# xrouting/xroute_env

Hardware: AMD Instinct MI355X
Metric: env-steps/sec (batched regions), ispd18_test1-sized regions (higher is better)
Workload: dtype u32 distances / i16 state / fp32 observation

## Files before the change

### xroute_env_amd/csrc/xr_kernels.hip

```cpp
#include <hip/hip_runtime.h>
#include <stdint.h>
#include <initializer_list>
#include <type_traits>

#include "xr_device.h"
#include "../../include/xroute_hip.h"

#define XR_FNV_PRIME 0x100000001b3ULL

__device__ __forceinline__ void fnv_mix(uint64_t& h, uint32_t w) { h = (h ^ (uint64_t)w) * XR_FNV_PRIME; }

__device__ __forceinline__ uint64_t splitmix64(uint64_t x) {
    x += 0x9E3779B97F4A7C15ULL;
    uint64_t z = x;
    z = (z ^ (z >> 30)) * 0xBF58476D1CE4E5B9ULL;
    z = (z ^ (z >> 27)) * 0x94D049BB133111EBULL;
    return z ^ (z >> 31);
}

__global__ void xr_ingest_kernel(const uint32_t* __restrict__ rec, int16_t* __restrict__ node_net,
                                 int16_t* __restrict__ owner0, int64_t total) {
    int64_t i = (int64_t)blockIdx.x * blockDim.x + threadIdx.x;
    const int64_t stride = (int64_t)gridDim.x * blockDim.x;
    for (; i < total; i += stride) {
// ... 1044 lines not shown
    __syncthreads();
    uint32_t v = 0, incl = 0;
    if (t < 256) {
        v = s_cnt[255 - t];
        incl = v;
        for (int o = 1; o < 64; o <<= 1) {
            const uint32_t u = __shfl_up(incl, o, 64);
            if ((t & 63) >= o) incl += u;
        }
        if ((t & 63) == 63) s_wsum[t >> 6] = incl;
    }
    __syncthreads();
    if (t < 256) {
        uint32_t base = 0;
        for (int w = 0; w < (t >> 6); w++) base += s_wsum[w];
        s_cnt[255 - t] = base + incl - v;
    }
    __syncthreads();
#pragma unroll
    for (int k = 0; k < 8; k++)
        if (cls[k] >= 0) order[atomicAdd(&s_cnt[cls[k]], 1u)] = e0 + t + k * 1024;
    for (int e = e0 + t + 8 * 1024; e < e1; e += 1024) order[atomicAdd(&s_cnt[xr_route_work_class(b, actions, e)], 1u)] = e;
}

template <bool LDS_DIST, int ZCH>
__global__ void __launch_bounds__(1024, 4) xr_route_kernel(XrBatchDev b, const int32_t* __restrict__ actions) {
    extern __shared__ __attribute__((aligned(16))) char smem[];
#ifdef XR_TIMELINE
    if (threadIdx.x == 0) {
        b.phase_cycles[(int64_t)blockIdx.x * 8 + 0] = (long long)wall_clock64();
        b.phase_cycles[(int64_t)blockIdx.x * 8 + 3] = (long long)__smid();
    }
#endif
    const int e_ = b.route_order ? b.route_order[blockIdx.x] : (int)blockIdx.x + b.env_base;
    xr_route_dispatch<LDS_DIST, ZCH>(b, e_, actions[e_], smem);
#ifdef XR_TIMELINE
    if (threadIdx.x == 0) b.phase_cycles[(int64_t)blockIdx.x * 8 + 1] = (long long)wall_clock64();
#endif
    if (b.obs_out) xr_obs_epilogue(b, e_, smem, b.obs_head_only != 0);
#ifdef XR_TIMELINE
    __syncthreads();
    if (threadIdx.x == 0) b.phase_cycles[(int64_t)blockIdx.x * 8 + 2] = (long long)wall_clock64();
#endif
}

template <int BT>
__global__ void __launch_bounds__(BT) xr_plan_kernel(XrBatchDev b, const int32_t* __restrict__ actions, uint32_t* __restrict__ next_queue,
                                                     int32_t* __restrict__ order) {
    __shared__ int s_wsum[BT / 64];
    __shared__ int s_base;
    const int tid = threadIdx.x, lane = tid & 63, wv = tid >> 6;
    const int e = b.env_base + blockIdx.x * BT + tid, e_end = XR_ENV_END(b);
    if (blockIdx.x == 0 && tid < 3 && next_queue) next_queue[tid] = 0u;
    int k = 0, r = 0;
    const uint64_t* lsrc = nullptr;
    int clear_bit = -1;
    bool was_reset = false;
    if (e < e_end) {
        const int nl = b.nlegal[e];
        r = b.env_region[e];
        was_reset = (nl == 0);
        if (nl == 0) {
            if (b.auto_reset) {
                if (b.env_replay[e] == b.max_route_count) r = (int)(((int64_t)r + b.n_envs) % b.n_regions);
                const XrRegionDev R = b.regions[r];
                lsrc = b.legal0 + R.legal0_off;
                k = R.nlegal0;
            }
        } else {
            const XrRegionDev R = b.regions[r];
            const int a = actions[e];
            lsrc = b.legal + (int64_t)e * b.legal_words;
            k = nl;
            if (a >= 1 && a <= R.n_nets && ((lsrc[(a - 1) >> 6] >> ((a - 1) & 63)) & 1ULL)) {
                clear_bit = a - 1;
                k = nl - 1;
            }
        }
        b.plan_region[e] = r;
    }
    int kskip = XR_SPLIT_KEEP(b, k);
    if (b.obs_incremental && e < e_end && !was_reset) {
        if (clear_bit < 0) kskip = k;
        else {
            int below = 0;
            for (int w = 0; w <= (clear_bit >> 6); w++) {
                uint64_t m = lsrc[w];
                if (w == (clear_bit >> 6)) m &= (1ULL << (clear_bit & 63)) - 1ULL;
                below += __popcll(m);
            }
            kskip = below;
        }
    }
    const int kw = k - kskip;
    int incl = kw;
#pragma unroll
    for (int d = 1; d < 64; d <<= 1) {
        const int t = __shfl_up(incl, d, 64);
        if (lane >= d) incl += t;
    }
    if (lane == 63) s_wsum[wv] = incl;
    __syncthreads();
    int woff = 0;
    for (int w = 0; w < wv; w++) woff += s_wsum[w];
    if (tid == BT - 1) s_base = (int)atomicAdd(&b.queue[2], (unsigned)(woff + incl));
    __syncthreads();
    const int off = s_base + woff + incl - kw;
    if (e < e_end) {
        int j = 0;
        for (int w = 0; w < b.legal_words && j < k; w++) {
            uint64_t m = lsrc[w];
            if (clear_bit >= 0 && (clear_bit >> 6) == w) m &= ~(1ULL << (clear_bit & 63));
            while (m) {
                const int bit = __ffsll((unsigned long long)m) - 1;
                m &= m - 1;
                if (j >= kskip) {
                    b.plan_units[off + j - kskip] = ((uint32_t)e << 14) | (uint32_t)j;
                    b.plan_unit_net[off + j - kskip] = (w << 6) + bit + 1;
                }
                j++;
            }
        }
    }
    if (order) {
        __shared__ uint32_t s_cnt[256];
        __shared__ uint32_t s_csum[4];
        if (tid < 256) s_cnt[tid] = 0;
        __syncthreads();
        const int cls = e < e_end ? xr_route_work_class(b, actions, e) : -1;
        if (cls >= 0) atomicAdd(&s_cnt[cls], 1u);
        __syncthreads();
        uint32_t v = 0, inc = 0;
        if (tid < 256) {
            v = s_cnt[255 - tid];
            inc = v;
            for (int o = 1; o < 64; o <<= 1) {
                const uint32_t u = __shfl_up(inc, o, 64);
                if (lane >= o) inc += u;
            }
            if (lane == 63) s_csum[wv] = inc;
        }
        __syncthreads();
        if (tid < 256) {
            uint32_t base = 0;
            for (int w = 0; w < wv; w++) base += s_csum[w];
            s_cnt[255 - tid] = base + inc - v;
        }
        __syncthreads();
        if (cls >= 0) order[atomicAdd(&s_cnt[cls], 1u)] = e;
    }
}

#define XR_NP_J 9
template <int J = XR_NP_J>
__device__ __forceinline__ void xr_unit_aligned(const XrBatchDev& b, int u, int t_lo = 0, int t_hi = 1 << 22) {
    const int tid = threadIdx.x;
    const uint32_t ent = b.plan_units[u];
    const int id = b.plan_unit_net[u];
    const int e = (int)(ent >> 14), rank = (int)(ent & 0x3FFFu);
    const XrRegionDev R = b.regions[b.plan_region[e]];
    const int N = R.N, Z = R.Z, Y = R.Y, X = R.X, YZ = Y * Z;
    const int16_t* __restrict__ nn = b.rg_node_net + R.node_off;
    float* __restrict__ out = b.obs_out + (int64_t)e * b.obs_stride + (int64_t)(2 + 7 * rank) * N;
    const int ngrp = N >> 2;
    const int ap_lo = b.net_csr[R.net_off + id], ap_hi = b.net_csr[R.net_off + id + 1];
    (void)nn; (void)X; (void)Y; (void)Z; (void)YZ;
    const int gend = min(ngrp, t_hi << 8);
    for (int g0 = t_lo << 8; g0 < gend; g0 += 256 * J) {
        unsigned bits[J];
#pragma unroll
        for (int j = 0; j < J; j++) bits[j] = 0;
        for (int i = ap_lo; i < ap_hi; i++) {
            const int v = b.ap_feat[R.ap_off + i];
            const int f = v & 0x7FFFFFFF;
            const unsigned m = (1u | (v < 0 ? 16u : 0u)) << (f & 3);
            const int g = (f >> 2) - g0 - tid;
#pragma unroll
            for (int j = 0; j < J; j++) bits[j] |= (g == j * 256) ? m : 0u;
        }
#pragma unroll
        for (int j = 0; j < J; j++) {
            const int g = g0 + j * 256 + tid;
            if (g < gend) {
                float* __restrict__ pp = out + ((int64_t)g << 2);
                const unsigned m0 = bits[j], m1 = bits[j] >> 4;
                float4 v0, v1;
                v0.x = (m0 & 1u) ? 1.f : 0.f; v0.y = (m0 & 2u) ? 1.f : 0.f; v0.z = (m0 & 4u) ? 1.f : 0.f; v0.w = (m0 & 8u) ? 1.f : 0.f;
                v1.x = (m1 & 1u) ? 1.f : 0.f; v1.y = (m1 & 2u) ? 1.f : 0.f; v1.z = (m1 & 4u) ? 1.f : 0.f; v1.w = (m1 & 8u) ? 1.f : 0.f;
                XR_ST4(pp, v0);
#pragma unroll
                for (int pl = 1; pl < 7; pl++) XR_ST4(pp + (int64_t)pl * N, v1);
            }
        }
    }
}

__global__ void __launch_bounds__(256) xr_netplane_kernel(XrBatchDev b) {
    const int total = (int)b.queue[2];
    for (int u = blockIdx.x; u < total; u += gridDim.x) xr_unit_aligned(b, u);
}

__device__ __forceinline__ void xr_unit_stream(const XrBatchDev& b, int u, uint32_t* s_m) {
    const int tid = threadIdx.x;
    const uint32_t ent = b.plan_units[u];
    const int id = b.plan_unit_net[u];
    const int e = (int)(ent >> 14), rank = (int)(ent & 0x3FFFu);
    const XrRegionDev R = b.regions[b.plan_region[e]];
    const int N = R.N, Z = R.Z, Y = R.Y, X = R.X, YZ = Y * Z;
    const int nwords = (N + 15) >> 4;
    (void)X; (void)Y; (void)Z; (void)YZ;
    const int ap_lo = b.net_csr[R.net_off + id], ap_hi = b.net_csr[R.net_off + id + 1];
    int my_ap = 0;
    const bool has_ap = ap_lo + tid < ap_hi;
    if (has_ap) my_ap = b.ap_feat[R.ap_off + ap_lo + tid];
    for (int w = tid; w <= nwords; w += 256) s_m[w] = 0u;
    xr_lds_barrier();
    if (has_ap) {
        const int f = my_ap & 0x7FFFFFFF;
        atomicOr(&s_m[f >> 4], (my_ap < 0 ? 3u : 1u) << ((f & 15) << 1));
    }
    xr_lds_barrier();
    float* __restrict__ run = b.obs_out + (int64_t)e * b.obs_stride + (int64_t)(2 + 7 * rank) * N;
    const int total = 7 * N;
    const int head = (int)((32u - (uint32_t)((reinterpret_cast<uintptr_t>(run) >> 2) & 31u)) & 31u);
    const int nslot = total > head ? (total - head) >> 2 : 0;
    const int piece = ((nslot + 7 * 256 - 1) / (7 * 256)) * 256;
    auto one = [&](int o) -> float {
        int pl = 0, f = o;
        while (f >= N) { f -= N; pl++; }
        return ((s_m[f >> 4] >> (((f & 15) << 1) + (pl ? 1 : 0))) & 1u) ? 1.f : 0.f;
    };
    int ppl[7], pnd[7];
#pragma unroll
    for (int p = 0; p < 7; p++) {
        int o = head + ((p * piece + tid) << 2), pl = 0;
        while (o >= N && pl < 7) { o -= N; pl++; }
        ppl[p] = pl; pnd[p] = o;
    }
    for (int it = 0; it < piece; it += 256) {
#pragma unroll
        for (int p = 0; p < 7; p++) {
            const int sl = p * piece + it + tid;
            if (sl < nslot) {
                const int f = pnd[p], pl = ppl[p];
                float4 v;
                if (f + 3 < N) {
                    const int bit = f << 1, w = bit >> 5;
                    const uint32_t m = __funnelshift_r(s_m[w], s_m[w + 1], bit & 31) >> (pl ? 1 : 0);
                    v.x = (m & 1u) ? 1.f : 0.f; v.y = (m & 4u) ? 1.f : 0.f; v.z = (m & 16u) ? 1.f : 0.f; v.w = (m & 64u) ? 1.f : 0.f;
                } else {
                    const int o = head + (sl << 2);
                    v.x = one(o); v.y = one(o + 1); v.z = one(o + 2); v.w = one(o + 3);
                }
                XR_ST4(run + head + (sl << 2), v);
            }
            int nf = pnd[p] + 1024;
            while (nf >= N) { nf -= N; ppl[p]++; }
            pnd[p] = nf;
        }
    }
    if (tid < head && tid < total) run[tid] = one(tid);
    const int tail0 = head + (nslot << 2);
    if (tid >= 64 && tail0 + (tid - 64) < total) run[tail0 + (tid - 64)] = one(tail0 + (tid - 64));
    xr_lds_barrier();
}

typedef unsigned xr_u4 __attribute__((ext_vector_type(4)));
#define XR_STU8(ptr, v) __builtin_nontemporal_store((v), reinterpret_cast<xr_u4*>(ptr))
__device__ __forceinline__ uint32_t xr_nib_bytes(uint32_t m) {
    return (m & 1u) | ((m & 2u) << 7) | ((m & 4u) << 14) | ((m & 8u) << 21);
}
__device__ __forceinline__ xr_u4 xr_bits_bytes16(uint32_t m) {
    return xr_u4{xr_nib_bytes(m), xr_nib_bytes(m >> 4), xr_nib_bytes(m >> 8), xr_nib_bytes(m >> 12)};
}
__device__ __forceinline__ uint32_t xr_pair_bytes(uint32_t m) {
    return (m & 1u) | ((m & 4u) << 6) | ((m & 16u) << 12) | ((m & 64u) << 18);
}
__device__ __forceinline__ uint32_t xr_obst_bytes4(uint32_t n0, uint32_t n1, uint32_t w0, uint32_t w1) {
    auto ob = [](uint32_t n, uint32_t w) -> uint32_t { return ((n & 0xFFFFu) == 0xFFFFu || (w & 0xFFFFu) != 0u) ? 1u : 0u; };
    return ob(n0, w0) | (ob(n0 >> 16, w0 >> 16) << 8) | (ob(n1, w1) << 16) | (ob(n1 >> 16, w1 >> 16) << 24);
}

__device__ __forceinline__ void xr_obs_head_u8(const XrBatchDev& b, int e, char* smem) {
    __syncthreads();
    const XrRegionDev R = b.regions[b.env_region[e]];
    int* s_ids = reinterpret_cast<int*>(smem);
    int* s_pref = s_ids + b.legal_words * 64;
    const int tid = threadIdx.x, nthr = (int)blockDim.x;
    int K;
    if (b.legal_words <= nthr) {
        const uint64_t my_m = tid < b.legal_words ? b.legal[(int64_t)e * b.legal_words + tid] : 0ull;
        K = xr_legal_ids_pre(my_m, b.legal_words, s_ids, s_pref);
    } else {
        K = xr_legal_ids(b.legal + (int64_t)e * b.legal_words, b.legal_words, s_ids, s_pref);
    }
    const int16_t* __restrict__ nn = b.rg_node_net + R.node_off;
    const int16_t* __restrict__ ow = b.owner + (int64_t)e * b.n_max;
    uint8_t* __restrict__ out = b.obs_out_u8 + (int64_t)e * b.obs_stride;
    const int N = R.N, total = 2 * N, nslot = total >> 4;
    auto one = [&](int o) -> uint32_t {
        if (o < N) return (nn[o] == -1 || ow[o] != 0) ? 1u : 0u;
        return o - N < K ? ((uint32_t)s_ids[o - N] & 0xFFu) : 0u;
    };
    for (int s = tid; s < nslot; s += nthr) {
        const int o = s << 4;
        xr_u4 v;
        if (o + 16 <= N) {
            const int4 a0 = *reinterpret_cast<const int4*>(nn + o), a1 = *reinterpret_cast<const int4*>(nn + o + 8);
            const int4 c0 = *reinterpret_cast<const int4*>(ow + o), c1 = *reinterpret_cast<const int4*>(ow + o + 8);
            v = xr_u4{xr_obst_bytes4(a0.x, a0.y, c0.x, c0.y), xr_obst_bytes4(a0.z, a0.w, c0.z, c0.w),
                      xr_obst_bytes4(a1.x, a1.y, c1.x, c1.y), xr_obst_bytes4(a1.z, a1.w, c1.z, c1.w)};
        } else if (o >= N + K) {
            v = xr_u4{0u, 0u, 0u, 0u};
        } else {
            uint32_t w[4];
#pragma unroll
            for (int q = 0; q < 4; q++)
                w[q] = one(o + 4 * q) | (one(o + 4 * q + 1) << 8) | (one(o + 4 * q + 2) << 16) | (one(o + 4 * q + 3) << 24);
            v = xr_u4{w[0], w[1], w[2], w[3]};
        }
        XR_STU8(out + o, v);
    }
    const int tail0 = nslot << 4;
    if (tid < total - tail0) out[tail0 + tid] = (uint8_t)one(tail0 + tid);
}

#define XR_NPU8_J 4
__device__ __forceinline__ void xr_unit_u8_aligned(const XrBatchDev& b, int u) {
    const int tid = threadIdx.x, nthr = (int)blockDim.x;
    const uint32_t ent = b.plan_units[u];
    const int id = b.plan_unit_net[u];
    const int e = (int)(ent >> 14), rank = (int)(ent & 0x3FFFu);
    const XrRegionDev R = b.regions[b.plan_region[e]];
    const int N = R.N;
    uint8_t* __restrict__ out = b.obs_out_u8 + (int64_t)e * b.obs_stride + (int64_t)(2 + 7 * rank) * N;
    const int ngrp = N >> 4;
    const int ap_lo = b.net_csr[R.net_off + id], ap_hi = b.net_csr[R.net_off + id + 1];
    for (int g0 = 0; g0 < ngrp; g0 += nthr * XR_NPU8_J) {
        uint32_t bits[XR_NPU8_J];
#pragma unroll
        for (int j = 0; j < XR_NPU8_J; j++) bits[j] = 0;
        for (int i = ap_lo; i < ap_hi; i++) {
            const int v = b.ap_feat[R.ap_off + i];
            const int f = v & 0x7FFFFFFF;
            const uint32_t m = (1u | (v < 0 ? 0x10000u : 0u)) << (f & 15);
            const int g = (f >> 4) - g0 - tid;
#pragma unroll
            for (int j = 0; j < XR_NPU8_J; j++) bits[j] |= (g == j * nthr) ? m : 0u;
        }
#pragma unroll
        for (int j = 0; j < XR_NPU8_J; j++) {
            const int g = g0 + j * nthr + tid;
            if (g < ngrp) {
                uint8_t* __restrict__ pp = out + ((int64_t)g << 4);
                const xr_u4 v0 = xr_bits_bytes16(bits[j]), v1 = xr_bits_bytes16(bits[j] >> 16);
                XR_STU8(pp, v0);
#pragma unroll
                for (int pl = 1; pl < 7; pl++) XR_STU8(pp + (int64_t)pl * N, v1);
            }
        }
    }
}

__device__ __forceinline__ void xr_unit_u8_stream(const XrBatchDev& b, int u, uint32_t* s_m) {
    const int tid = threadIdx.x, nthr = (int)blockDim.x;
    const uint32_t ent = b.plan_units[u];
    const int id = b.plan_unit_net[u];
    const int e = (int)(ent >> 14), rank = (int)(ent & 0x3FFFu);
    const XrRegionDev R = b.regions[b.plan_region[e]];
    const int N = R.N;
    const int nwords = (N + 15) >> 4;
    const int ap_lo = b.net_csr[R.net_off + id], ap_hi = b.net_csr[R.net_off + id + 1];
    for (int w = tid; w <= nwords; w += nthr) s_m[w] = 0u;
    xr_lds_barrier();
    for (int i = ap_lo + tid; i < ap_hi; i += nthr) {
        const int v = b.ap_feat[R.ap_off + i];
        const int f = v & 0x7FFFFFFF;
        atomicOr(&s_m[f >> 4], (v < 0 ? 3u : 1u) << ((f & 15) << 1));
    }
    xr_lds_barrier();
    uint8_t* __restrict__ run = b.obs_out_u8 + (int64_t)e * b.obs_stride + (int64_t)(2 + 7 * rank) * N;
    const int total = 7 * N;
    const int head = min(total, (int)((128u - (uint32_t)(reinterpret_cast<uintptr_t>(run) & 127u)) & 127u));
    const int nslot = (total - head) >> 4;
    auto one = [&](int o) -> uint32_t {
        const int pl = o / N, f = o - pl * N;
        return (s_m[f >> 4] >> (((f & 15) << 1) + (pl ? 1 : 0))) & 1u;
    };
    for (int sl = tid; sl < nslot; sl += nthr) {
        const int o = head + (sl << 4);
        const int pl = o / N, f = o - pl * N;
        xr_u4 v;
        if (f + 15 < N) {
            const int bit = f << 1, w = bit >> 5;
            const uint32_t m = __funnelshift_r(s_m[w], s_m[w + 1], bit & 31) >> (pl ? 1 : 0);
            v = xr_u4{xr_pair_bytes(m), xr_pair_bytes(m >> 8), xr_pair_bytes(m >> 16), xr_pair_bytes(m >> 24)};
        } else {
            uint32_t q4[4];
#pragma unroll
            for (int q = 0; q < 4; q++)
                q4[q] = one(o + 4 * q) | (one(o + 4 * q + 1) << 8) | (one(o + 4 * q + 2) << 16) | (one(o + 4 * q + 3) << 24);
            v = xr_u4{q4[0], q4[1], q4[2], q4[3]};
        }
        XR_STU8(run + o, v);
    }
    for (int i = tid; i < head; i += nthr) run[i] = (uint8_t)one(i);
    const int tail0 = head + (nslot << 4);
    for (int i = tail0 + tid; i < total; i += nthr) run[i] = (uint8_t)one(i);
    xr_lds_barrier();
}

__global__ void __launch_bounds__(256) xr_obs_u8_kernel(XrBatchDev b, uint8_t* __restrict__ out, int64_t env_stride, int env_lo) {
    extern __shared__ __attribute__((aligned(16))) char smem[];
    int* s_ids = reinterpret_cast<int*>(smem);
    int* s_pref = s_ids + b.legal_words * 64;
    const int e = env_lo + blockIdx.y;
    const XrRegionDev R = b.regions[b.env_region[e]];
    const int N = R.N;
    const int64_t slot0 = (int64_t)blockIdx.x * blockDim.x;
    if ((slot0 << 4) >= (int64_t)(2 + 7 * (int64_t)R.n_nets) * N) return;
    const int K = xr_legal_ids(b.legal + (int64_t)e * b.legal_words, b.legal_words, s_ids, s_pref);
    const int64_t total = (int64_t)(2 + 7 * (int64_t)K) * N;
    const int64_t o = (slot0 + threadIdx.x) << 4;
    if (o >= total) return;
    XrStateSrc src{b.rg_node_net + R.node_off, b.owner + (int64_t)e * b.n_max};
    uint8_t* __restrict__ row = out + (int64_t)blockIdx.y * env_stride;
    int p = (int)(o / N), f = (int)(o - (int64_t)p * N);
    uint32_t w[4] = {0u, 0u, 0u, 0u};
    const int cnt = total - o < 16 ? (int)(total - o) : 16;
    for (int j = 0; j < cnt; j++) {
        float obst; int apnet; bool adj;
        xr_node_features(src, f, R.X, R.Y, R.Z, N, obst, apnet, adj);
        uint32_t v;
        if (p == 0) v = obst != 0.f ? 1u : 0u;
        else if (p == 1) v = f < K ? ((uint32_t)s_ids[f] & 0xFFu) : 0u;
        else {
            const int pi = p - 2, i = pi / 7, c = pi - 7 * i;
            v = (apnet != 0 && apnet == s_ids[i] && (c == 0 || adj)) ? 1u : 0u;
        }
        w[j >> 2] |= v << ((j & 3) << 3);
        if (++f == N) { f = 0; ++p; }
    }
    if (cnt == 16) {
        XR_STU8(row + o, (xr_u4{w[0], w[1], w[2], w[3]}));
    } else {
        for (int j = 0; j < cnt; j++) row[o + j] = (uint8_t)(w[j >> 2] >> ((j & 3) << 3));
    }
}

constexpr int XR_QUEUE_BATCH = 1;
constexpr int XR_TICKET_TILES = 3;
static_assert(XR_TICKET_TILES >= 1 && XR_TICKET_TILES <= XR_NP_J, "a slab is one pass of xr_unit_aligned");
__device__ __forceinline__ void xr_queue_first(int G, int sh, int& first_r, int& first_u) {
    if (sh < 0) { first_r = G; first_u = 0; return; }
    first_r = ((G >> (sh + 1)) << sh) + min(G & ((2 << sh) - 1), 1 << sh);
    first_u = G - first_r;
}

__global__ void __launch_bounds__(256) xr_unit_helper_kernel(XrBatchDev b) {
    __shared__ int s_u;
    const int total = (int)b.queue[2];
    int first_r, first_u;
    xr_queue_first(b.queue_grid, b.queue_skip_shift, first_r, first_u);
    for (;;) {
        if (threadIdx.x == 0) s_u = first_u + (int)atomicAdd(&b.queue[1], 1u);
        __syncthreads();
        const int u = s_u;
        __syncthreads();
        if (u >= total) break;
        xr_unit_aligned(b, u);
    }
}

__global__ void __launch_bounds__(256) xr_netplane_stream_kernel(XrBatchDev b) {
    extern __shared__ __attribute__((aligned(16))) char smem[];
    const int total = (int)b.queue[2];
    for (int u = blockIdx.x; u < total; u += gridDim.x) xr_unit_stream(b, u, reinterpret_cast<uint32_t*>(smem));
}

constexpr int XR_QUEUE_WAVES_PER_SIMD = 4;
template <bool LDS_DIST, int ZCH, bool U8>
__device__ __forceinline__ void xr_step_queue_body(XrBatchDev& b, const int32_t* __restrict__ actions, char* smem) {
    __shared__ int s_task;
    const int tid = threadIdx.x;
    const int B = XR_ENV_END(b) - b.env_base;
    const int units = (int)b.queue[2];
    int S = 1;
    if (!U8 && b.obs_vec4 == 1 && b.queue_slab_tickets) {
        S = ((b.n_max + 1023) / 1024 + XR_TICKET_TILES - 1) / XR_TICKET_TILES;
        if ((int64_t)units * S > 0x7FF00000LL) S = 1;
    }
    const int total = units * S;
    const bool claim_late = S > 1;
    const int quota = S * max(1, (int)(((int64_t)units * b.queue_quota_pm) / (1000 * (int64_t)B)));
    bool routes_left = true, units_left = total > 0;
    bool skip_route = b.queue_skip_shift >= 0 && ((blockIdx.x >> b.queue_skip_shift) & 1) != 0;
    int first_r = 0, first_u = 0, my_first = -1;
    const bool unit_first = skip_route;
    {
        const int sh = b.queue_skip_shift, G = (int)gridDim.x, i = (int)blockIdx.x;
        xr_queue_first(G, sh, first_r, first_u);
        my_first = sh < 0 ? i : ((i >> (sh + 1)) << sh) + (i & ((1 << sh) - 1));
    }
#ifdef XR_TIMELINE
    long long tl_start = wall_clock64(), tl_route = 0, tl_unit = 0, tl_last_route = 0;
    int tl_nr = 0, tl_nu = 0;
#define XR_TL_NOW() wall_clock64()
#endif
    while (routes_left || units_left) {
        if (routes_left && !skip_route) {
            if (tid == 0) {
                const int t = (my_first >= 0 && !unit_first) ? my_first : first_r + (int)atomicAdd(&b.queue[0], 1u);
                s_task = (t < B && b.route_order) ? b.route_order[t] : b.env_base + t;
            }
            if (!unit_first) my_first = -1;
            xr_lds_barrier();
            const int e = s_task;
            xr_lds_barrier();
            if (e < b.env_base + B) {
#ifdef XR_TIMELINE
                const long long t0 = XR_TL_NOW();
#endif
                xr_route_dispatch<LDS_DIST, ZCH>(b, e, actions[e], smem);
                if constexpr (U8) xr_obs_head_u8(b, e, smem);
                else xr_obs_epilogue(b, e, smem, true);
                xr_lds_barrier();
#ifdef XR_TIMELINE
                tl_last_route = XR_TL_NOW(); tl_route += tl_last_route - t0; tl_nr++;
#endif
            } else {
                routes_left = false;
            }
        }
        skip_route = false;
        if (units_left) {
            const int nb = routes_left ? max(1, quota / XR_QUEUE_BATCH) : (1 << 30);
            unsigned nx = 0;
            const unsigned ubase = (unsigned)first_u * (unsigned)XR_QUEUE_BATCH;
            auto claim = [&]() -> unsigned { return ubase + atomicAdd(&b.queue[1], (unsigned)XR_QUEUE_BATCH); };
            if (tid == 0) nx = (my_first >= 0 && unit_first) ? (unsigned)my_first * (unsigned)XR_QUEUE_BATCH : claim();
            if (unit_first) my_first = -1;
            for (int i = 0; i < nb; i++) {
                if (tid == 0) s_task = (int)nx;
                xr_lds_barrier();
                const int u0 = s_task;
                xr_lds_barrier();
                if (u0 >= total) { units_left = false; break; }
                if (!claim_late && tid == 0 && i + 1 < nb) nx = claim();
#ifdef XR_TIMELINE
                const long long t0 = XR_TL_NOW();
#endif
                const int u1 = min(u0 + XR_QUEUE_BATCH, total);
                for (int u = u0; u < u1; u++) {
                    if constexpr (U8) {
                        if (b.obs_vec4 == 1) xr_unit_u8_aligned(b, u);
                        else xr_unit_u8_stream(b, u, reinterpret_cast<uint32_t*>(smem));
                    } else {
                        if (b.obs_vec4 == 1) {
                            if (S > 1) {
                                const int uu = u / S, p = u - uu * S;
                                xr_unit_aligned<XR_TICKET_TILES>(b, uu, p * XR_TICKET_TILES, (p + 1) * XR_TICKET_TILES);
                            } else xr_unit_aligned(b, u);
                        } else xr_unit_stream(b, u, reinterpret_cast<uint32_t*>(smem));
                    }
                }
#ifdef XR_TIMELINE
                tl_unit += XR_TL_NOW() - t0; tl_nu += u1 - u0;
#endif
                if (claim_late && tid == 0 && i + 1 < nb) nx = claim();
            }
            xr_lds_barrier();
        }
    }
#ifdef XR_TIMELINE
    if (tid == 0 && (int)blockIdx.x < B) {
        long long* o = b.phase_cycles + (int64_t)blockIdx.x * 8;
        o[0] = tl_start; o[1] = XR_TL_NOW(); o[2] = tl_route; o[3] = tl_unit; o[4] = tl_nr; o[5] = tl_nu; o[6] = tl_last_route; o[7] = 1;
    }
#endif
}

template <bool LDS_DIST, int ZCH>
__global__ void __launch_bounds__(1024, XR_QUEUE_WAVES_PER_SIMD) xr_step_queue_kernel(XrBatchDev b, const int32_t* __restrict__ actions) {
    extern __shared__ __attribute__((aligned(16))) char smem[];
    xr_step_queue_body<LDS_DIST, ZCH, false>(b, actions, smem);
}

template <bool LDS_DIST, int ZCH>
__global__ void __launch_bounds__(1024, XR_QUEUE_WAVES_PER_SIMD) xr_step_queue_u8_kernel(XrBatchDev b, const int32_t* __restrict__ actions) {
    extern __shared__ __attribute__((aligned(16))) char smem[];
    xr_step_queue_body<LDS_DIST, ZCH, true>(b, actions, smem);
}

template <bool LDS_DIST, int ZCH>
__global__ void xr_order_kernel(XrBatchDev b, const int32_t* __restrict__ orders, int stride,
                                int32_t* __restrict__ net_stats) {
    extern __shared__ __attribute__((aligned(16))) char smem[];
    const int e = blockIdx.x;
    const int tid = threadIdx.x;
    xr_env_reset(b, e, 0, 0);
    __syncthreads();
    int st_acc = 0, plen_acc = 0, sweeps_acc = 0;
    const int32_t* __restrict__ ord = orders + (int64_t)e * stride;
    for (int k = 0; k < stride; k++) {
        const int a = ord[k];
// ... 265 lines not shown
    hipError_t e = hipFuncGetAttributes(&attr, fn);
    if (e != hipSuccess) return e;
    *static_lds = attr.sharedSizeBytes;
    return hipOccupancyMaxActiveBlocksPerMultiprocessor(wg_per_cu, fn, v.threads, v.lds_bytes);
}

hipError_t xr_launch_step_queue(const XrBatchDev* b, const int32_t* actions, XrRouteVariant v, int blocks, hipStream_t st) {
    const dim3 g(blocks), t(v.threads);
    xr_with_variant(v.lds_dist, v.zch, [&](auto L, auto Z) {
        if (b->obs_out_u8) hipLaunchKernelGGL((xr_step_queue_u8_kernel<L.value, Z.value>), g, t, v.lds_bytes, st, *b, actions);
        else hipLaunchKernelGGL((xr_step_queue_kernel<L.value, Z.value>), g, t, v.lds_bytes, st, *b, actions);
    });
    return hipGetLastError();
}

hipError_t xr_lookahead_occupancy(XrRouteVariant v, int* wg_per_cu) {
    const void* fn = xr_with_variant(v.lds_dist, v.zch, [](auto L, auto Z) { return reinterpret_cast<const void*>(&xr_lookahead_kernel<L.value, Z.value>); });
    return hipOccupancyMaxActiveBlocksPerMultiprocessor(wg_per_cu, fn, v.threads, v.lds_bytes);
}

hipError_t xr_launch_lookahead_plan(const XrBatchDev* b, int env_lo, int rows, const uint64_t* cand_mask, int32_t* out, double* reward_out, int k_cap,
                                    int k_max, uint32_t* tasks, uint32_t* ctr, uint32_t* next_ctr, hipStream_t st) {
    hipLaunchKernelGGL(xr_lookahead_plan_kernel, dim3((rows + 3) / 4), dim3(256), 0, st, *b, env_lo, rows, cand_mask, out, reward_out, k_cap, k_max, tasks, ctr,
                       next_ctr);
    return hipGetLastError();
}

hipError_t xr_launch_lookahead(const XrBatchDev* src, const XrBatchDev* shadow, int env_lo, const uint32_t* tasks, uint32_t* ctr, int32_t* out,
                               double* reward_out, int k_cap, int k_max, XrRouteVariant v, int blocks, hipStream_t st) {
    const dim3 g(blocks), t(v.threads);
    xr_with_variant(v.lds_dist, v.zch, [&](auto L, auto Z) {
        hipLaunchKernelGGL((xr_lookahead_kernel<L.value, Z.value>), g, t, v.lds_bytes, st, *src, *shadow, env_lo, tasks, ctr, out, reward_out, k_cap, k_max);
    });
    return hipGetLastError();
}

hipError_t xr_launch_line(const XrLineLaunch* l, hipStream_t st) {
    const XrRouteVariant& v = l->v;
    const dim3 g(l->blocks), t(v.threads);
    switch (l->kind) {
    case XR_LINE_POLICY:
        xr_with_variant(v.lds_dist, v.zch, [&](auto L, auto Z) {
            hipLaunchKernelGGL((xr_rollout_kernel<L.value, Z.value>), g, t, v.lds_bytes, st, *l->src, *l->shadow, l->env_lo, l->n_tasks, l->per_row, l->policy, l->seed,
                               l->prefix, l->prefix_stride, l->max_plies, l->ctr, l->next_ctr, l->out, l->return_out, l->hash_out, l->order_out, l->k_cap);
        });
        break;
    case XR_LINE_PEEK:
        xr_with_variant(v.lds_dist, v.zch, [&](auto L, auto Z) {
            hipLaunchKernelGGL((xr_peek_kernel<L.value, Z.value>), g, t, v.lds_bytes, st, *l->src, *l->shadow, l->env_lo, l->n_tasks, l->per_row, l->prefix,
                               l->prefix_stride, l->max_plies, l->ctr, l->next_ctr, l->rows, l->row_bytes, l->region_base, l->out, l->return_out, l->hash_out,
                               l->order_out, l->k_cap);
        });
        break;
    case XR_LINE_WEIGHTED:
        xr_with_variant(v.lds_dist, v.zch, [&](auto L, auto Z) {
            hipLaunchKernelGGL((xr_rollout_weighted_kernel<L.value, Z.value>), g, t, v.lds_bytes, st, *l->src, *l->shadow, l->env_lo, l->n_tasks, l->per_row, l->seed,
                               l->prefix, l->prefix_stride, l->max_plies, l->ctr, l->next_ctr, l->out, l->return_out, l->hash_out, l->order_out, l->k_cap, l->weights,
                               l->weights_k_cap);
        });
        break;
    }
    return hipGetLastError();
}

hipError_t xr_launch_weighted_actions(const XrBatchDev* b, const int32_t* weights, int k_cap, int32_t* actions, uint64_t seed, hipStream_t st) {
    const int n = XR_ENV_END(*b) - b->env_base;
    hipLaunchKernelGGL(xr_weighted_action_kernel, dim3((n + 3) / 4), dim3(256), 0, st, *b, weights, k_cap, actions, seed);
    return hipGetLastError();
}

hipError_t xr_launch_branch(const XrSlotRows* env, const XrSlotRows* stg, int env_lo, int rows, const int32_t* parent, int n_max, int path_cap,
                            int legal_words, int chunks, hipStream_t st) {
    const dim3 g(rows, chunks), t(256);
    hipLaunchKernelGGL(xr_branch_kernel<0>, g, t, 0, st, *env, *stg, env_lo, rows, parent, n_max, path_cap, legal_words);
    hipLaunchKernelGGL(xr_branch_kernel<1>, g, t, 0, st, *env, *stg, env_lo, rows, parent, n_max, path_cap, legal_words);
    return hipGetLastError();
}

hipError_t xr_launch_tree_reset(const XrBatchDev* src, const XrTreeDev* t, int rows, hipStream_t st) {
    hipLaunchKernelGGL(xr_tree_reset_kernel, dim3(rows), dim3(64), 0, st, *src, *t);
    return hipGetLastError();
}

hipError_t xr_launch_tree_select(const XrBatchDev* src, const XrTreeDev* t, int rows, int wave, hipStream_t st) {
    const size_t lds = (size_t)src->legal_words * sizeof(uint64_t) + (2 * (size_t)t->k_cap + 1) * sizeof(int32_t);
    hipLaunchKernelGGL(xr_tree_select_kernel, dim3(rows), dim3(64), lds, st, *src, *t, wave);
    return hipGetLastError();
}

hipError_t xr_launch_tree_backup(const XrBatchDev* src, const XrTreeDev* t, int rows, int wave, int last, hipStream_t st) {
    hipLaunchKernelGGL(xr_tree_backup_kernel, dim3(rows), dim3(64), 0, st, *src, *t, wave, last);
    return hipGetLastError();
}

hipError_t xr_launch_tree_keep_begin(const XrBatchDev* src, const XrTreeDev* t, const XrTreeKeepDev* k, int rows, hipStream_t st) {
    hipLaunchKernelGGL(xr_tree_keep_begin_kernel, dim3(rows), dim3(64), 0, st, *src, *t, *k);
    return hipGetLastError();
}

hipError_t xr_launch_tree_eval_open(const XrBatchDev* src, const XrTreeEvalDev* t, const float* root_prior, int rows, hipStream_t st) {
    hipLaunchKernelGGL(xr_tree_eval_open_kernel, dim3(rows), dim3(64), 0, st, *src, *t, root_prior);
    return hipGetLastError();
}

hipError_t xr_launch_tree_eval_select(const XrTreeEvalDev* t, int32_t* paths_out, int32_t* leaf_out, int rows, hipStream_t st) {
    const size_t lds = (size_t)t->legal_words * sizeof(uint64_t) + (2 * (size_t)t->k_cap + 1) * sizeof(int32_t);
    hipLaunchKernelGGL(xr_tree_eval_select_kernel, dim3(rows), dim3(64), lds, st, *t, paths_out, leaf_out);
    return hipGetLastError();
}

hipError_t xr_launch_tree_eval_backup(const XrTreeEvalDev* t, const double* value, const float* leaf_prior, int sims, int32_t* visits_out, double* value_out,
                                      int32_t* info_out, int32_t* best_order_out, double* best_return_out, double* returns_out, int rows, hipStream_t st) {
    hipLaunchKernelGGL(xr_tree_eval_backup_kernel, dim3(rows), dim3(64), 0, st, *t, value, leaf_prior, sims, visits_out, value_out, info_out, best_order_out,
                       best_return_out, returns_out);
    return hipGetLastError();
}

hipError_t xr_launch_route_order(const XrBatchDev* b, const int32_t* actions, int32_t* order, hipStream_t st) {
    hipLaunchKernelGGL(xr_route_order_kernel, dim3(1), dim3(1024), 0, st, *b, actions, order);
    return hipGetLastError();
}

hipError_t xr_launch_plan(const XrBatchDev* b, const int32_t* actions, uint32_t* next_queue, int32_t* order, int* order_done, hipStream_t st) {
    if (order_done) *order_done = 0;
    const int n = XR_ENV_END(*b) - b->env_base;
    if (order && n <= 1024) {
        hipLaunchKernelGGL(xr_plan_kernel<1024>, dim3(1), dim3(1024), 0, st, *b, actions, next_queue, order);
        if (order_done) *order_done = 1;
    } else {
        hipLaunchKernelGGL(xr_plan_kernel<256>, dim3((n + 255) / 256), dim3(256), 0, st, *b, actions, next_queue, (int32_t*)nullptr);
    }
    return hipGetLastError();
}

hipError_t xr_launch_netplanes(const XrBatchDev* b, int blocks, int aligned, hipStream_t st) {
    if (aligned) hipLaunchKernelGGL(xr_netplane_kernel, dim3(blocks), dim3(256), 0, st, *b);
    else hipLaunchKernelGGL(xr_netplane_stream_kernel, dim3(blocks), dim3(256), (size_t)(((b->n_max + 15) / 16 + 2) * 4), st, *b);
    return hipGetLastError();
}

hipError_t xr_launch_random_actions(const XrBatchDev* b, int32_t* actions, uint64_t seed, hipStream_t st) {
    const int n = XR_ENV_END(*b) - b->env_base;
    hipLaunchKernelGGL(xr_random_action_kernel, dim3((n + 255) / 256), dim3(256), 0, st, *b, actions, seed);
    return hipGetLastError();
}

hipError_t xr_launch_obs(const XrBatchDev* b, float* out, int64_t env_stride, int env_lo, int env_hi, int n_max_nodes, int vec4, hipStream_t st) {
    if (env_hi <= env_lo) return hipSuccess;
    const size_t lds = (size_t)(b->legal_words * 64 + b->legal_words + 1) * sizeof(int);
    for (int lo = env_lo; lo < env_hi; lo += 32768) {
        const int cnt = (env_hi - lo) < 32768 ? (env_hi - lo) : 32768;
        float* o = out + (int64_t)(lo - env_lo) * env_stride;
        if (vec4 == 1) {
            const int chunks = (n_max_nodes + 1023) / 1024;
            hipLaunchKernelGGL(xr_obs_kernel<4>, dim3(chunks, cnt), dim3(256), lds, st, *b, o, env_stride, lo);
        } else if (vec4 == 2) {
            const size_t lds2 = (size_t)(b->legal_words * 64 + ((b->legal_words + 1 + 3) & ~3)) * sizeof(int) + (size_t)b->n_max * 2;
            hipLaunchKernelGGL(xr_obs_stream_kernel, dim3(cnt), dim3(256), lds2, st, *b, o, env_stride, lo);
        } else {
            const int chunks = (n_max_nodes + 255) / 256;
            hipLaunchKernelGGL(xr_obs_kernel<1>, dim3(chunks, cnt), dim3(256), lds, st, *b, o, env_stride, lo);
        }
    }
    return hipGetLastError();
}

hipError_t xr_launch_obs_u8(const XrBatchDev* b, uint8_t* out, int64_t env_stride, int env_lo, int env_hi, int n_max_nodes, int k_max, hipStream_t st) {
    if (env_hi <= env_lo) return hipSuccess;
    const size_t lds = (size_t)(b->legal_words * 64 + b->legal_words + 1) * sizeof(int);
    const int chunks = (int)(((2 + 7 * (int64_t)k_max) * n_max_nodes + 4095) / 4096);
    if (chunks <= 0) return hipSuccess;
    for (int lo = env_lo; lo < env_hi; lo += 32768) {
        const int cnt = (env_hi - lo) < 32768 ? (env_hi - lo) : 32768;
        hipLaunchKernelGGL(xr_obs_u8_kernel, dim3(chunks, cnt), dim3(256), lds, st, *b, out + (int64_t)(lo - env_lo) * env_stride, env_stride, lo);
    }
    return hipGetLastError();
}

hipError_t xr_launch_unit_helpers(const XrBatchDev* b, int blocks, hipStream_t st) {
    hipLaunchKernelGGL(xr_unit_helper_kernel, dim3(blocks), dim3(256), 0, st, *b);
    return hipGetLastError();
}

hipError_t xr_launch_netplanes_pairs(const XrBatchDev* b, const int32_t* pair_region, const int32_t* pair_net, int n_pairs,
                                     float* out, int64_t pair_stride, int vec4, hipStream_t st) {
    if (n_pairs <= 0) return hipSuccess;
    hipLaunchKernelGGL(xr_netplanes_pairs_kernel, dim3(n_pairs), dim3(256), 0, st, *b, pair_region, pair_net, out, pair_stride, vec4);
    return hipGetLastError();
}

hipError_t xr_launch_guide_masks(const XrBatchDev* b, uint8_t* masks, int k_max, hipStream_t st) {
    if (b->n_regions <= 0 || k_max <= 0) return hipSuccess;
    for (int r0 = 0; r0 < b->n_regions; r0 += 32768) {
        hipLaunchKernelGGL(xr_guide_mask_kernel, dim3(k_max, (b->n_regions - r0) < 32768 ? (b->n_regions - r0) : 32768), dim3(256), 0, st, *b, masks, r0);
        const hipError_t e = hipGetLastError();
        if (e != hipSuccess) return e;
    }
    return hipSuccess;
}

hipError_t xr_launch_ingest_state(const XrBatchDev* b, const int16_t* owner_in, const uint64_t* legal_in, const int32_t* cum_in, hipStream_t st) {
    if (b->n_envs <= 0) return hipSuccess;
    hipLaunchKernelGGL(xr_ingest_state_kernel, dim3(b->n_envs), dim3(256), 0, st, *b, owner_in, legal_in, cum_in);
    return hipGetLastError();
}

hipError_t xr_launch_pack_state(const XrBatchDev* b, uint8_t* rows, int64_t row_bytes, int region_base, hipStream_t st) {
    if (b->n_envs <= 0) return hipSuccess;
    hipLaunchKernelGGL(xr_pack_state_kernel, dim3(b->n_envs), dim3(256), 0, st, *b, rows, row_bytes, region_base);
    return hipGetLastError();
}

hipError_t xr_launch_expand_state(const XrBatchDev* b, const uint8_t* rows, int64_t row_bytes, int n_rows, float* head, int64_t head_stride,
                                  int32_t* nlegal_out, int32_t* region_out, int vec4, hipStream_t st) {
    if (n_rows <= 0) return hipSuccess;
    const size_t lds = (size_t)(b->legal_words * 64 + b->legal_words + 1) * sizeof(int);
    hipLaunchKernelGGL(xr_expand_state_kernel, dim3(n_rows), dim3(256), lds, st, *b, rows, row_bytes, head, head_stride, nlegal_out, region_out, vec4);
    return hipGetLastError();
}

hipError_t xr_launch_obs_records(const uint32_t* rec, int X, int Y, int Z, const int32_t* nets, int K, float* out,
                                 int vec4, hipStream_t st) {
    const int N = X * Y * Z;
    if (N <= 0) return hipSuccess;
    const size_t lds = (size_t)(K > 0 ? K : 1) * sizeof(int);
    if (vec4)
        hipLaunchKernelGGL(xr_obs_records_kernel<4>, dim3((N + 1023) / 1024), dim3(256), lds, st, rec, X, Y, Z, nets, K, out);
    else
        hipLaunchKernelGGL(xr_obs_records_kernel<1>, dim3((N + 255) / 256), dim3(256), lds, st, rec, X, Y, Z, nets, K, out);
    return hipGetLastError();
}

}
```

Baseline: 2.392 million.

## Split vec4 observation kernel into per-net slab blocks across a 3D grid

Replaces the vec4 observation launch with a new slab kernel on a 3D grid of node slabs × net groups × envs. Each block writes either the base state planes or one legal net's seven planes for a three-tile slab, reusing the aligned net-plane routine, which is factored out into a shared helper. The goal is to spread the per-net plane writes over many more blocks and so raise parallelism. The cost is many empty blocks that early-exit, plus each block recomputing the popcount and legal-id prefix.

After: 2.391 million (median of 2 runs). About the same (-0.0%).

```diff
diff --git a/xroute_env_amd/csrc/xr_kernels.hip b/xroute_env_amd/csrc/xr_kernels.hip
--- a/xroute_env_amd/csrc/xr_kernels.hip
+++ b/xroute_env_amd/csrc/xr_kernels.hip
@@ -1220,19 +1220,12 @@
 }
 
 #define XR_NP_J 9
-template <int J = XR_NP_J>
-__device__ __forceinline__ void xr_unit_aligned(const XrBatchDev& b, int u, int t_lo = 0, int t_hi = 1 << 22) {
+template <int J>
+__device__ __forceinline__ void xr_net_slab(const XrBatchDev& b, const XrRegionDev& R, float* __restrict__ out, int id, int t_lo, int t_hi) {
     const int tid = threadIdx.x;
-    const uint32_t ent = b.plan_units[u];
-    const int id = b.plan_unit_net[u];
-    const int e = (int)(ent >> 14), rank = (int)(ent & 0x3FFFu);
-    const XrRegionDev R = b.regions[b.plan_region[e]];
-    const int N = R.N, Z = R.Z, Y = R.Y, X = R.X, YZ = Y * Z;
-    const int16_t* __restrict__ nn = b.rg_node_net + R.node_off;
-    float* __restrict__ out = b.obs_out + (int64_t)e * b.obs_stride + (int64_t)(2 + 7 * rank) * N;
+    const int N = R.N;
     const int ngrp = N >> 2;
     const int ap_lo = b.net_csr[R.net_off + id], ap_hi = b.net_csr[R.net_off + id + 1];
-    (void)nn; (void)X; (void)Y; (void)Z; (void)YZ;
     const int gend = min(ngrp, t_hi << 8);
     for (int g0 = t_lo << 8; g0 < gend; g0 += 256 * J) {
         unsigned bits[J];
@@ -1261,6 +1254,15 @@
             }
         }
     }
+}
+
+template <int J = XR_NP_J>
+__device__ __forceinline__ void xr_unit_aligned(const XrBatchDev& b, int u, int t_lo = 0, int t_hi = 1 << 22) {
+    const uint32_t ent = b.plan_units[u];
+    const int id = b.plan_unit_net[u];
+    const int e = (int)(ent >> 14), rank = (int)(ent & 0x3FFFu);
+    const XrRegionDev R = b.regions[b.plan_region[e]];
+    xr_net_slab<J>(b, R, b.obs_out + (int64_t)e * b.obs_stride + (int64_t)(2 + 7 * rank) * R.N, id, t_lo, t_hi);
 }
 
 __global__ void __launch_bounds__(256) xr_netplane_kernel(XrBatchDev b) {
@@ -1519,6 +1521,31 @@
 constexpr int XR_QUEUE_BATCH = 1;
 constexpr int XR_TICKET_TILES = 3;
 static_assert(XR_TICKET_TILES >= 1 && XR_TICKET_TILES <= XR_NP_J, "a slab is one pass of xr_unit_aligned");
+
+__global__ void __launch_bounds__(256) xr_obs_slab_kernel(XrBatchDev b, float* __restrict__ out, int64_t env_stride, int env_lo) {
+    extern __shared__ __attribute__((aligned(16))) char smem[];
+    int* s_ids = reinterpret_cast<int*>(smem);
+    int* s_pref = s_ids + b.legal_words * 64;
+    const int e = env_lo + blockIdx.z;
+    const XrRegionDev R = b.regions[b.env_region[e]];
+    const int t_lo = blockIdx.x * XR_TICKET_TILES, t_hi = t_lo + XR_TICKET_TILES;
+    if ((t_lo << 10) >= R.N) return;
+    const uint64_t* __restrict__ lw = b.legal + (int64_t)e * b.legal_words;
+    int left = 0;
+    for (int w = 0; w < b.legal_words; w++) left += __popcll(lw[w]);
+    if ((int)blockIdx.y > left) return;
+    float* __restrict__ row = out + (int64_t)blockIdx.z * env_stride;
+    const int K = xr_legal_ids(lw, b.legal_words, s_ids, s_pref);
+    for (int j = blockIdx.y; j <= K; j += gridDim.y) {
+        if (j == 0) {
+            XrStateSrc src{b.rg_node_net + R.node_off, b.owner + (int64_t)e * b.n_max};
+            for (int t = t_lo; t < t_hi; t++) xr_obs_write<XrStateSrc, 4>(src, R.X, R.Y, R.Z, R.N, s_ids, K, row, t << 10, 0);
+        } else {
+            xr_net_slab<XR_TICKET_TILES>(b, R, row + (int64_t)(2 + 7 * (j - 1)) * R.N, s_ids[j - 1], t_lo, t_hi);
+        }
+    }
+}
+
 __device__ __forceinline__ void xr_queue_first(int G, int sh, int& first_r, int& first_u) {
     if (sh < 0) { first_r = G; first_u = 0; return; }
     first_r = ((G >> (sh + 1)) << sh) + min(G & ((2 << sh) - 1), 1 << sh);
@@ -2090,8 +2117,9 @@
         const int cnt = (env_hi - lo) < 32768 ? (env_hi - lo) : 32768;
         float* o = out + (int64_t)(lo - env_lo) * env_stride;
         if (vec4 == 1) {
-            const int chunks = (n_max_nodes + 1023) / 1024;
-            hipLaunchKernelGGL(xr_obs_kernel<4>, dim3(chunks, cnt), dim3(256), lds, st, *b, o, env_stride, lo);
+            const int slabs = ((n_max_nodes + 1023) / 1024 + XR_TICKET_TILES - 1) / XR_TICKET_TILES;
+            const int groups = 1 + (b->legal_words * 64 < 65534 ? b->legal_words * 64 : 65534);
+            hipLaunchKernelGGL(xr_obs_slab_kernel, dim3(slabs, groups, cnt), dim3(256), lds, st, *b, o, env_stride, lo);
         } else if (vec4 == 2) {
             const size_t lds2 = (size_t)(b->legal_words * 64 + ((b->legal_words + 1 + 3) & ~3)) * sizeof(int) + (size_t)b->n_max * 2;
             hipLaunchKernelGGL(xr_obs_stream_kernel, dim3(cnt), dim3(256), lds2, st, *b, o, env_stride, lo);
```
